# mpkuse/cerebro

Measured on AMD Instinct MI355X. Metric: loop-queries/sec (ticks of 3 descriptors vs 4096-D x 1M DB), higher is better.
Workload: dtype f64

## Files before the change

### cerebro_amd/csrc/chip_api.hip

```cpp
#include "chip_internal.h"
#include <cmath>
#include <cstdlib>
#include <cstring>
#include <memory>
#include <new>

using namespace chip;

extern "C" {

const char *chip_strerror(int status)
{
    switch (status) {
        case CHIP_OK: return "ok";
        case CHIP_ERR_INVALID_ARG: return "invalid argument";
        case CHIP_ERR_NO_DEVICE: return "no usable HIP device";
        case CHIP_ERR_HIP: return "HIP runtime error (see chip_last_hip_error)";
        case CHIP_ERR_OOM: return "out of device memory";
        case CHIP_ERR_NOT_F32: return "descriptor value not exactly representable as float32";
        case CHIP_ERR_NONFINITE: return "NaN/Inf in descriptor";
        case CHIP_ERR_RANGE: return "index / length out of range";
        case CHIP_ERR_UNSUPPORTED: return "unsupported configuration";
        case CHIP_ERR_TOO_FEW_POINTS: return "fewer than 20 correspondences";
        case CHIP_ERR_BUSY: return "async slot busy or empty";
// ... 140 lines not shown
    if (c->s_pnp) (void)hipStreamDestroy(c->s_pnp);
    delete c;
}

void scan_read_knobs(Ctx *c)
{
    c->scan_block = env_int("CHIP_SCAN_BLOCK", 0);
    if (c->scan_block != 256 && c->scan_block != 512 && c->scan_block != 768 && c->scan_block != 1024) c->scan_block = 0;
    c->scan_blocks_per_cu = env_int("CHIP_SCAN_BPC", 2);
    if (c->scan_blocks_per_cu < 1) c->scan_blocks_per_cu = 1;
    c->scan_variant = env_int("CHIP_SCAN_VARIANT", 0);
    c->scan_rows = env_int("CHIP_SCAN_ROWS", 0);
    c->scan_claim = env_int("CHIP_SCAN_CLAIM", -1);
    c->tick_same_stream = env_int("CHIP_TICK_SAME_STREAM", 1) != 0;
    c->scan_short_bpc = env_int("CHIP_SCAN_SHORT_BPC", 1);
    c->scan_plain_bytes = (double)env_int("CHIP_SCAN_PLAIN_MIB", 768) * 1024 * 1024;
    c->scan_half_bytes = (double)env_int("CHIP_SCAN_HALF_MIB", 192) * 1024 * 1024;
    c->scan_sync_plain_bytes = (double)env_int("CHIP_SCAN_SYNC_PLAIN_MIB", 4096) * 1024 * 1024;
    c->scan_overlap_bytes = (double)env_int("CHIP_SCAN_OVERLAP_GIB", 8) * 1024 * 1024 * 1024;
    c->scan_reserve = env_int("CHIP_SCAN_RESERVE", c->nranks > 1 ? 4 : 0);
    c->max_grid = 512;
    c->scan_streams = env_int("CHIP_SCAN_STREAMS", c->nranks > 1 ? 2 : 4);
    c->tick_fused = env_int("CHIP_TICK_FUSED", 1) != 0;
}

static int create_impl(chip_ctx *c, int64_t capacity_hint, int elem)
{
    hipDeviceProp_t prop;
    CHIP_HIP(c, hipGetDeviceProperties(&prop, c->device));
    c->n_cus = prop.multiProcessorCount;
    std::strncpy(c->arch, prop.gcnArchName, sizeof(c->arch) - 1);
    if (std::strncmp(c->arch, "gfx950", 6) != 0 && !std::getenv("CHIP_ALLOW_ANY_ARCH")) return CHIP_ERR_NO_DEVICE;

    c->segs.reserve(kMaxSegs);

    CHIP_HIP(c, hipStreamCreateWithFlags(&c->s_query, hipStreamNonBlocking));
    CHIP_HIP(c, hipStreamCreateWithFlags(&c->s_append, hipStreamNonBlocking));
    CHIP_HIP(c, hipStreamCreateWithFlags(&c->s_pnp, hipStreamNonBlocking));
    int rc = c->seg_table_dev.alloc(c, kMaxSegs);
    if (rc == CHIP_OK) rc = configure_storage(c, elem);
    if (rc != CHIP_OK) return rc;
    c->stage_bytes = 64ull << 20;
    if (c->stage_bytes < (size_t)c->D * 8 * 64) c->stage_bytes = (size_t)c->D * 8 * 64;
    rc = c->stage_dev.alloc(c, c->stage_bytes);
    if (rc == CHIP_OK) rc = c->flags_dev.alloc(c, 1);
    if (rc == CHIP_OK) rc = c->flags_host.alloc(c, 1);
// ... 333 lines not shown
    scan_args_db(c, &a);
    a.K = K;
    a.partial = c->partial_dev[b];
    for (int t = 0; t < T; t++) {
        a.k[t] = parked[t].k;
        if (a.k[t] > a.n_rows) a.n_rows = a.k[t];
        for (int i = 0; i < 3; i++) a.q[3 * t + i] = parked[t].q[i];
    }
    const int grid = scan_multi_grid(c);
    double E = 0.0;
    int e = 0;
    if (prefilter) {
        std::lock_guard<std::mutex> lk(c->mu);
        if (halfq) {
            e = halfq_exponent(c->row_norm_max);
            a.q_up = std::ldexp(1.0f, e);
            a.s_up = std::ldexp(1.0, e);
            a.s_down = std::ldexp(1.0, -e);
            E = halfq_error_bound(c->D, c->row_norm_max, e);
        } else {
            E = prefilter_error_bound(c->D, c->row_norm_max);
        }
    }
    if (hipEventQuery(c->ev_merged[b]) != hipSuccess) CHIP_HIP(c, hipStreamWaitEvent(c->s_scan, c->ev_merged[b], 0));
    hipEvent_t e1 = nullptr;
    int rc = c->prof_on ? prof_begin(c, c->s_scan, (double)a.n_rows * c->D * c->elem, &e1) : CHIP_OK;
    if (rc == CHIP_OK)
        rc = halfq ? launch_scan_halfq(c, c->s_scan, a, grid) : prefilter ? launch_scan_prefilter(c, c->s_scan, a, grid) : launch_scan_multi(c, c->s_scan, a, T, grid);
    if (rc != CHIP_OK) return rc;
    if (e1) CHIP_HIP(c, hipEventRecord(e1, c->s_scan));
    CHIP_HIP(c, hipEventRecord(c->ev_scan[b], c->s_scan));
    c->pass_ev = c->ev_scan[b];
    c->pass_shared = true;
    c->pass_no++;
    CHIP_HIP(c, hipStreamWaitEvent(c->s_query, c->ev_scan[b], 0));
    chip_topk_entry *exact = c->partial_dev[b] + (size_t)kPassMaxTicks * grid * 3 * K;
    if (prefilter) {
        RescoreArgs ra{};
        ra.seg_table = a.seg_table; ra.seg_shift = a.seg_shift; ra.seg_mask = a.seg_mask; ra.D = a.D; ra.K = K;
        ra.in = c->partial_dev[b]; ra.n_lists = grid; ra.wpb = 8;
        ra.E = E;
        ra.out = exact;
        for (int t = 0; t < T; t++) {
            const Ctx::ParkedTick &pt = parked[t];
            Slot &s = *pt.slot;
            ra.k[t] = pt.k;
            for (int i = 0; i < 3; i++) { ra.q[3 * t + i] = s.pf_q[i] = pt.q[i]; s.cert_host[i] = 0; }
            ra.cert[t] = s.cert_dev;
            s.prefilter = true; s.pf_k = pt.k; s.pf_p = pt.p;
        }
        rc = launch_rescore(c, c->s_query, ra, T);
        if (rc != CHIP_OK) return rc;
        Ctx::LastPass &lp = c->last_pass;
        lp.family = halfq ? CHIP_SCAN_FAMILY_HALFQ : CHIP_SCAN_FAMILY_PREFILTER;
        lp.ticks = T; lp.grid = grid; lp.wpb = ra.wpb; lp.K = K; lp.e = e; lp.ring = b; lp.E = E;
        for (int t = 0; t < T; t++) { lp.k[t] = parked[t].k; lp.cert[t] = parked[t].slot->cert_host; }
    }
    if (halfq) {
        PassMergeArgs m{};
        m.in = exact;
        m.K = K;
        for (int t = 0; t < T; t++) {
            const MergeArgs mt = merge_args(exact + (size_t)t * 3 * K, 1, K, nullptr, parked[t].slot->rec.dev(), parked[t].l, &parked[t].p);
            m.result[t] = mt.result; m.l[t] = mt.l; m.locality[t] = mt.locality; m.thresh[t] = mt.thresh;
        }
        rc = launch_pass_merge(c, c->s_query, m, T);
        if (rc != CHIP_OK) return rc;
    }
    for (int t = 0; t < T; t++) {
        const Ctx::ParkedTick &pt = parked[t];
        if (halfq) rc = CHIP_OK;
        else if (prefilter) rc = launch_merge(c, c->s_query, merge_args(exact + (size_t)t * 3 * K, 1, K, nullptr, pt.slot->rec.dev(), pt.l, &pt.p), 3);
        else rc = launch_merge(c, c->s_query, merge_args(c->partial_dev[b] + (size_t)t * grid * 3 * K, grid, K, nullptr, pt.slot->rec.dev(), pt.l, &pt.p), 3);
        if (rc != CHIP_OK) return rc;
        CHIP_HIP(c, hipEventRecord(pt.slot->done, c->s_query));
        pt.slot->wait_ev = pt.slot->done;
        pt.slot->state = SlotState::Event;
        pt.slot->pass_no = c->pass_no;
    }
    CHIP_HIP(c, hipEventRecord(c->ev_merged[b], c->s_query));
    c->coalesce_passes++;
    c->coalesce_ticks += T;
    if (prefilter) { c->prefilter_passes++; c->prefilter_ticks += T; }
    return CHIP_OK;
}

int coalesce_flush(Ctx *c)
{
    const int T = c->n_parked;
    if (T == 0) return CHIP_OK;
    c->n_parked = 0;
    const Ctx::ParkedTick &p0 = c->parked[0];
    int rc;
    if (T == kHalfqTicks && !scan_halfq_usable(c)) {
        rc = coalesce_submit(c, 0, kMultiMaxTicks);
        if (rc == CHIP_OK) rc = coalesce_submit(c, kMultiMaxTicks, T - kMultiMaxTicks);
    } else if (T == kPrefilterTicks && !scan_prefilter_usable(c)) {
        const Ctx::ParkedTick &pl = c->parked[T - 1];
        rc = coalesce_submit(c, 0, T - 1);
        if (rc == CHIP_OK) rc = tick_submit(c, pl.k, pl.l, &pl.p, pl.q, false, *pl.slot);
    } else {
        rc = T == 1 ? tick_submit(c, p0.k, p0.l, &p0.p, p0.q, false, *p0.slot) : coalesce_submit(c, 0, T);
    }
// ... 927 lines not shown
```

### cerebro_amd/csrc/chip_internal.h

```cpp
#pragma once
#include <hip/hip_runtime.h>
#include <cstdint>
#include <mutex>
#include <utility>
#include <condition_variable>
#include <vector>
#include "../../include/cerebro_hip.h"

namespace chip {

constexpr int kWave = 64;
constexpr int kMaxSegs = 4096;
constexpr int64_t kSegBytesTarget = 512ll << 20;

struct ScanArgs {
    const void *const *seg_table;
    int32_t seg_shift;
    int64_t seg_mask;
    int64_t n_rows;
    int32_t D;
    int32_t K;
    const void *q[CHIP_MAX_NQ];
    int64_t idx_mul, idx_add;
    chip_topk_entry *partial;
// ... 21 lines not shown
    uint64_t seq_ptr;
    uint64_t seq_val;
    uint32_t dyn_claim;
    uint32_t tail;
};
static_assert(sizeof(ResidentCmd) == 64, "one cache line, one PCIe read");
constexpr uint32_t kResidentLeave = 0xffffffffu;

struct ResidentArgs {
    ScanArgs base;
    const uint32_t *cmd_host;
    uint32_t *cmd_dev;
    unsigned long long *exit_host;
    unsigned long long instance;
    unsigned long long lease_ticks;
    uint32_t done;
    uint32_t direct;
};

constexpr int kMultiMaxTicks = 3;
constexpr int kPrefilterTicks = 4;
constexpr int kRescoreCap = 32;
constexpr int kHalfqTicks = 5;
constexpr int kPassMaxTicks = kHalfqTicks;
struct PassArgs {
    const void *const *seg_table;
    int32_t seg_shift;
    int64_t seg_mask;
    int64_t n_rows;
    int32_t D;
    int32_t K;
    int64_t k[kPassMaxTicks];
    const void *q[3 * kPassMaxTicks];
    chip_topk_entry *partial;
    float q_up;
    double s_down, s_up;
};
struct RescoreArgs {
    const void *const *seg_table;
    int32_t seg_shift;
    int64_t seg_mask;
    int32_t D;
    int32_t K;
    const chip_topk_entry *in;
    int32_t n_lists;
    int32_t wpb;
    int64_t k[kPassMaxTicks];
    const void *q[3 * kPassMaxTicks];
    double E;
    chip_topk_entry *out;
    uint32_t *cert[kPassMaxTicks];
};
struct PassMergeArgs {
    const chip_topk_entry *in;
    int32_t K;
    chip_tick_result *result[kPassMaxTicks];
    int64_t l[kPassMaxTicks];
    int32_t locality[kPassMaxTicks];
    double thresh[kPassMaxTicks];
// ... 218 lines not shown

    DevBuf<char> stage_dev;
    size_t stage_bytes = 0;
    DevBuf<uint32_t> flags_dev;
    PinnedBuf<uint32_t> flags_host;
    DevBuf<unsigned long long> norm2_dev;
    PinnedBuf<unsigned long long> norm2_host;
    double row_norm_max = 0.0;

    static constexpr int kRing = 64;
    hipStream_t s_scan = nullptr;
    hipStream_t s_scan2 = nullptr;
    hipStream_t s_scan_x[2] = {};
    uint64_t n_same_stream = 0;
    DevBuf<chip_topk_entry> partial_dev[kRing];
    int32_t partial_lists[kRing] = {};
    hipEvent_t ev_scan[kRing] = {};
    hipEvent_t ev_merged[kRing] = {};
    DevBuf<int32_t> tickets_dev;
    PinnedBuf<unsigned long long> seq_all;
    unsigned long long tick_seq = 0;
    bool tick_poll = true;
    bool tick_fused = true;
    Resident res;
    uint64_t n_enqueued = 0;
    int32_t max_grid = 0;
    PinnedBuf<chip_topk_entry> topk;

    DevBuf<char> qvec_dev;
    DevBuf<double> scores_dev;
    DevBuf<unsigned long long> stamps_dev;

    std::vector<char> qconv;
    int64_t cap_hint = 0;
    int32_t group_transport = 0;
    mutable int last_comm = 0;
    int32_t comm_init_abandoned = 0;
    Exchange *xchg = nullptr;
    Group *group = nullptr;
    Ctx *parent = nullptr;
    Slot slots[CHIP_MAX_INFLIGHT];
    int64_t last_l = 0;

    struct ParkedTick { Slot *slot; int64_t k, l; chip_dot_params p; const void *q[3]; };
    int32_t coalesce_max = 5;
    bool coalesce_force = false;
// ... 239 lines not shown
```

### cerebro_amd/csrc/kernels.hip

```cpp
#include "chip_internal.h"
#include "topk_merge.h"
#include <cmath>
#include <type_traits>

namespace chip {

typedef float f32x4 __attribute__((ext_vector_type(4)));
typedef double f64x2 __attribute__((ext_vector_type(2)));

template <typename T> struct Vec16;
template <> struct Vec16<float> { typedef f32x4 type; static constexpr int N = 4; };
template <> struct Vec16<double> { typedef f64x2 type; static constexpr int N = 2; };

template <typename V>
__device__ __forceinline__ const __attribute__((address_space(1))) V *as_global(const V *p)
{
    return (const __attribute__((address_space(1))) V *)p;
}

template <typename V>
__device__ __forceinline__ V stream_load(const V *p)
{
    return __builtin_nontemporal_load(as_global(p));
}
// ... 90 lines not shown
template <typename T>
__device__ __forceinline__ const T *row_base(const ScanArgs &a, int64_t r)
{
    return static_cast<const T *>(a.seg_table[r >> a.seg_shift]) + (r & a.seg_mask) * (int64_t)a.D;
}

__device__ __forceinline__ void wave_topk_offer(double s, int64_t gi, int K, int lane, double &my_s, int64_t &my_i, double &thr_s, int64_t &thr_i)
{
    if (key_gt(s, gi, thr_s, thr_i)) {
        const bool worse = key_gt(s, gi, my_s, my_i);
        const unsigned long long m = __ballot(worse) & ((1ull << K) - 1ull);
        const int pos = __builtin_ctzll(m);
        const double up_s = __shfl_up(my_s, 1, 64);
        const int64_t up_i = __shfl_up(my_i, 1, 64);
        if (lane < K) {
            if (lane > pos) { my_s = up_s; my_i = up_i; }
            else if (lane == pos) { my_s = s; my_i = gi; }
        }
        thr_s = __shfl(my_s, K - 1, 64);
        thr_i = __shfl(my_i, K - 1, 64);
    }
}

template <int NQ, typename OutOf>
__device__ __forceinline__ void block_merge_cand(const chip_topk_entry *cand, int K, int lane, int wave, int wpb, OutOf out_of)
{
    __syncthreads();
    for (int q = wave; q < NQ; q += wpb) {
        const int ncand = wpb * K;
        double cs[4];
        int64_t ci[4];
#pragma unroll
        for (int h = 0; h < 4; h++) {
            const int c = lane + 64 * h;
            if (c < ncand) {
                const chip_topk_entry t = cand[((c / K) * NQ + q) * K + (c % K)];
                cs[h] = t.score;
                ci[h] = t.idx;
            } else { cs[h] = -INFINITY; ci[h] = -1; }
        }
        chip_topk_entry *outp = out_of(q);
        for (int j = 0; j < K; j++) {
            double bs = cs[0];
            int64_t bi = ci[0];
#pragma unroll
            for (int h = 1; h < 4; h++)
                if (key_gt(cs[h], ci[h], bs, bi)) { bs = cs[h]; bi = ci[h]; }
#pragma unroll
            for (int m = 32; m >= 1; m >>= 1) {
                const double os = __shfl_xor(bs, m, 64);
                const int64_t oi = __shfl_xor(bi, m, 64);
                if (key_gt(os, oi, bs, bi)) { bs = os; bi = oi; }
            }
#pragma unroll
            for (int h = 0; h < 4; h++)
                if (ci[h] == bi && cs[h] == bs) { cs[h] = -INFINITY; ci[h] = -1; }
            if (lane == 0) { chip_topk_entry t; t.score = bs; t.idx = bi; outp[j] = t; }
        }
    }
}

template <int NQ, typename OutOf>
__device__ __forceinline__ void block_merge_store(char *smem, const double (&my_s)[NQ], const int64_t (&my_i)[NQ],
                                                  int K, int lane, int wave, int wpb, OutOf out_of)
{
    __syncthreads();
    chip_topk_entry *cand = reinterpret_cast<chip_topk_entry *>(smem);
    if (lane < K) {
#pragma unroll
        for (int q = 0; q < NQ; q++) {
            chip_topk_entry t;
            t.score = my_s[q];
            t.idx = my_i[q];
            cand[(wave * NQ + q) * K + lane] = t;
        }
    }
    block_merge_cand<NQ>(cand, K, lane, wave, wpb, out_of);
}

template <typename T, typename Args>
// ... 44 lines not shown
    __syncthreads();

    double my_s[NQ], thr_s[NQ];
    int64_t my_i[NQ], thr_i[NQ];
#pragma unroll
    for (int q = 0; q < NQ; q++) { my_s[q] = -INFINITY; my_i[q] = -1; thr_s[q] = -INFINITY; thr_i[q] = -1; }

    const int64_t tw = (int64_t)gridDim.x * wpb;
    for (int64_t r = (int64_t)blockIdx.x * wpb + wave; r < a.n_rows; r += tw) {
        const T *row[1] = {row_base<T>(a, r)};
        double acc[1][NQ];
        rows_dot<T, NQ, U, FULL, NT, 1>(row, qs, D, lane, acc);
#pragma unroll
        for (int q = 0; q < NQ; q++) acc[0][q] = butterfly_sum(acc[0][q]);
        const int64_t gi = r * a.idx_mul + a.idx_add;
#pragma unroll
        for (int q = 0; q < NQ; q++) wave_topk_offer(acc[0][q], gi, K, lane, my_s[q], my_i[q], thr_s[q], thr_i[q]);
    }

    block_merge_store<NQ>(smem, my_s, my_i, K, lane, wave, wpb, [&](int q) { return a.partial + ((int64_t)blockIdx.x * NQ + q) * K; });
}

constexpr int kMultiR = 4, kMultiU = 4, kMultiBlock = 512;

constexpr int kMultiVgprBase = 192;
#if defined(__HIP_DEVICE_COMPILE__) && !defined(__gfx950__)
#error "the shared-pass kernels name physical VGPRs: gfx950 (MI355X) only -- build with --offload-arch=gfx950"
#endif
#define CHIP_PASS_SLOTS_192_255                                                                                                         \
    "v192", "v193", "v194", "v195", "v196", "v197", "v198", "v199", "v200", "v201", "v202", "v203", "v204", "v205", "v206", "v207",     \
    "v208", "v209", "v210", "v211", "v212", "v213", "v214", "v215", "v216", "v217", "v218", "v219", "v220", "v221", "v222", "v223",     \
    "v224", "v225", "v226", "v227", "v228", "v229", "v230", "v231", "v232", "v233", "v234", "v235", "v236", "v237", "v238", "v239",     \
    "v240", "v241", "v242", "v243", "v244", "v245", "v246", "v247", "v248", "v249", "v250", "v251", "v252", "v253", "v254", "v255"
#define CHIP_PASS_SLOTS_160_191                                                                                                         \
    "v160", "v161", "v162", "v163", "v164", "v165", "v166", "v167", "v168", "v169", "v170", "v171", "v172", "v173", "v174", "v175",     \
    "v176", "v177", "v178", "v179", "v180", "v181", "v182", "v183", "v184", "v185", "v186", "v187", "v188", "v189", "v190", "v191"
#define CHIP_PASS_SLOTS_144_159                                                                                                         \
    "v144", "v145", "v146", "v147", "v148", "v149", "v150", "v151", "v152", "v153", "v154", "v155", "v156", "v157", "v158", "v159"
__host__ __device__ constexpr int pass_row_slot(int u, int rr) { return kMultiVgprBase + 4 * (u * kMultiR + rr); }
__host__ __device__ constexpr int pass_query_slot(int ng, int u, int g) { return kMultiVgprBase - 4 * kMultiU * ng + 4 * (u * ng + g); }
__host__ __device__ constexpr int pass_vgpr_base(int max_ng) { return kMultiVgprBase - 4 * kMultiU * max_ng; }

template <int N, int I = 0, class F>
__device__ __forceinline__ void static_for(F &&f)
{
    if constexpr (I < N) {
// ... 137 lines not shown
            if (lane > pos) me = up;
            else if (lane == pos) { me.score = s; me.idx = gi; }
            list[lane] = me;
        }
        if constexpr (SCALED) thr_s = (S)(readlane_f64(me.score, K - 1) * sc_up);
        else thr_s = (S)readlane_f64(me.score, K - 1);
    }
}

template <typename T, int NS>
__device__ __forceinline__ void pass_stage_copy(T *qs, const PassArgs &a, int tid)
{
    typedef typename Vec16<T>::type V;
    constexpr int N = Vec16<T>::N;
    const int D = a.D;
    for (int e = tid * N; e < D; e += blockDim.x * N) {
        V w[NS];
#pragma unroll
        for (int q = 0; q < NS; q++) w[q] = *as_global(reinterpret_cast<const V *>(static_cast<const T *>(a.q[q]) + e));
#pragma unroll
        for (int q = 0; q < NS; q++) *reinterpret_cast<V *>(qs + q * D + e) = w[q];
    }
}

template <class P>
__device__ __forceinline__ void shared_pass(const PassArgs &a)
{
    typedef typename P::Elem T;
    typedef typename P::Score S;
    typedef typename P::Staged Q;
    constexpr int NQ = P::NQ, NG = P::NG, NS = NQ - NG, R = kMultiR, U = kMultiU, N = Vec16<T>::N;
    constexpr int BATCH = 64 * N * U;
    static_assert(pass_vgpr_base(NG) >= P::kVgprBase && pass_row_slot(U - 1, R - 1) + 4 <= 256, "load slots inside the asm's share of the register file");
    static_assert(NG >= 0 && NS >= 2 && P::L == U * (R + NG) && P::L <= 64, "at least two staged queries (the LDS read-ahead), vmcnt counts to 63");
    extern __shared__ __attribute__((aligned(16))) char smem[];
    asm volatile("" ::: CHIP_PASS_SLOTS_192_255);
    if constexpr (P::kVgprBase <= 160) asm volatile("" ::: CHIP_PASS_SLOTS_160_191);
    if constexpr (P::kVgprBase <= 144) asm volatile("" ::: CHIP_PASS_SLOTS_144_159);
    Q *qs = reinterpret_cast<Q *>(smem);
    const int D = a.D;
    const int K = a.K;
    const int tid = threadIdx.x;
    const int lane = tid & 63;
    const int wave = __builtin_amdgcn_readfirstlane(tid >> 6);
    const int wpb = blockDim.x >> 6;

// ... 67 lines not shown
            if (hit) {
#pragma unroll
                for (int q = 0; q < NQ; q++) {
                    asm volatile("" : "+v"(s[q]));
                    if (__ballot(s[q] >= thr_s[q])) {
#pragma unroll
                        for (int rr = 0; rr < R; rr++) {
                            const int64_t r = rbase + ((int64_t)group * R + rr) * tw;
                            if (r < a.n_rows && r < a.k[q / 3]) pass_offer<S, P::kScaled>(lane_value(s[q], 16 * rr), r, K, lane, mylists + q * K, thr_s[q], P::kScaled ? a.s_down : 1.0, P::kScaled ? a.s_up : 1.0);
                        }
                    }
                }
            }
#pragma unroll
            for (int rr = 0; rr < R; rr++)
#pragma unroll
                for (int q = 0; q < NQ; q++) acc[rr][q] = P::zero();
            b = 0;
            group++;
        }
    }
    asm volatile("s_waitcnt vmcnt(0)" ::: "memory");

    block_merge_cand<NQ>(lists, K, lane, wave, wpb,
                         [&](int q) { return a.partial + (((int64_t)(q / 3) * gridDim.x + blockIdx.x) * 3 + q % 3) * K; });
}

constexpr int kSharedMaxNG = 2;
constexpr int kSharedF64MaxTicks = 2;
template <typename T, int NTICKS, int NG_, int MAX_NG>
struct PassF64 {
    typedef T Elem;
    typedef T Staged;
    typedef double Score;
    typedef double Acc;
    static constexpr bool kScaled = false;
    static constexpr int NQ = 3 * NTICKS, NG = NG_, NS = NQ - NG, R = kMultiR, U = kMultiU, L = U * (R + NG), kVgprBase = pass_vgpr_base(MAX_NG);
    static __device__ __forceinline__ void stage(T *qs, const PassArgs &a, int tid) { pass_stage_copy<T, NS>(qs, a, tid); }
    static __device__ __forceinline__ Acc zero() { return 0.0; }
    static __device__ __forceinline__ double lane_sum(Acc v) { return v; }
    static __device__ __forceinline__ void batch(Acc (&acc)[R][NQ], const T *qv, int D, uint32_t voff, const T *const (&row)[R], const T *const (&qg)[NG > 0 ? NG : 1])
    {
        typedef typename Vec16<T>::type V;
        constexpr int N = Vec16<T>::N, SS = U * NS;
        V w[SS];
        w[0] = *reinterpret_cast<const V *>(qv);
        w[1] = *reinterpret_cast<const V *>(qv + D);
        double x[R][N];
        static_for<U * NQ>([&](auto sc) CHIP_INLINE_LAMBDA {
            constexpr int u = sc / NQ, q = sc % NQ;
            if constexpr (q == 0)
                static_for<R>([&](auto rr) CHIP_INLINE_LAMBDA {
                    slot_take<pass_row_slot(u, rr), L - 1>(x[rr]);
                    slot_issue<pass_row_slot(u, rr), u * 1024, true>(voff, row[rr]);
                });
            double wd[N];
            if constexpr (q < NS) {
                constexpr int i = u * NS + q;
                if constexpr (i + 2 < SS) w[i + 2] = *reinterpret_cast<const V *>(qv + ((i + 2) % NS) * D + ((i + 2) / NS) * (64 * N));
// ... 25 lines not shown
    shared_pass<PassF64<double, NTICKS, NG, kSharedMaxNG>>(a);
}

constexpr int kPrefilterMaxNG = 3;
typedef float f32x2 __attribute__((ext_vector_type(2)));

template <int REG>
__device__ __forceinline__ void prefilter_fma(f32x2 &acc, f32x2 w)
{
    asm volatile("v_pk_fma_f32 %0, v[%2:%3], %1, %0" : "+v"(acc) : "v"(w), "n"(REG), "n"(REG + 1));
}
template <int REG, int QREG>
__device__ __forceinline__ void prefilter_fma_slot(f32x2 &acc)
{
    asm volatile("v_pk_fma_f32 %0, v[%1:%2], v[%3:%4], %0" : "+v"(acc) : "n"(REG), "n"(REG + 1), "n"(QREG), "n"(QREG + 1));
}

template <int NG_>
struct PassF32 {
    typedef float Elem;
    typedef float Staged;
    typedef float Score;
    typedef f32x2 Acc;
    static constexpr bool kScaled = false;
    static constexpr int NQ = 3 * kPrefilterTicks, NG = NG_, NS = NQ - NG, R = kMultiR, U = kMultiU, L = U * (R + NG), kVgprBase = pass_vgpr_base(kPrefilterMaxNG);
    static __device__ __forceinline__ void stage(float *qs, const PassArgs &a, int tid) { pass_stage_copy<float, NS>(qs, a, tid); }
    static __device__ __forceinline__ Acc zero() { return (f32x2){0.0f, 0.0f}; }
    static __device__ __forceinline__ float lane_sum(Acc v) { return v[0] + v[1]; }
    static __device__ __forceinline__ void batch(Acc (&acc)[R][NQ], const float *qv, int D, uint32_t voff, const float *const (&row)[R], const float *const (&qg)[NG > 0 ? NG : 1])
    {
        constexpr int SS = U * NS;
        f32x4 w[SS];
        w[0] = *reinterpret_cast<const f32x4 *>(qv);
        w[1] = *reinterpret_cast<const f32x4 *>(qv + D);
        static_for<U>([&](auto uc) CHIP_INLINE_LAMBDA {
            constexpr int u = uc;
            slot_wait<L - R>();
            static_for<NS>([&](auto qc) CHIP_INLINE_LAMBDA {
                constexpr int q = qc, i = u * NS + q;
                if constexpr (i + 2 < SS) w[i + 2] = *reinterpret_cast<const f32x4 *>(qv + ((i + 2) % NS) * D + ((i + 2) / NS) * 256);
                const f32x2 wl = __builtin_shufflevector(w[i], w[i], 0, 1), wh = __builtin_shufflevector(w[i], w[i], 2, 3);
                static_for<R>([&](auto rr) CHIP_INLINE_LAMBDA { prefilter_fma<pass_row_slot(u, rr)>(acc[rr][q], wl); });
                static_for<R>([&](auto rr) CHIP_INLINE_LAMBDA { prefilter_fma<pass_row_slot(u, rr) + 2>(acc[rr][q], wh); });
                __builtin_amdgcn_sched_barrier(0);
            });
            static_for<NG>([&](auto gc) CHIP_INLINE_LAMBDA {
                constexpr int g = gc, QR = pass_query_slot(NG, u, g);
                slot_wait<L - R - 1 - g>();
                static_for<R>([&](auto rr) CHIP_INLINE_LAMBDA { prefilter_fma_slot<pass_row_slot(u, rr), QR>(acc[rr][NS + g]); });
                static_for<R>([&](auto rr) CHIP_INLINE_LAMBDA { prefilter_fma_slot<pass_row_slot(u, rr) + 2, QR + 2>(acc[rr][NS + g]); });
            });
            slots_issue_kib<u, NG>(voff, row, qg);
        });
    }
};

template <int NG>
__global__ __launch_bounds__(kMultiBlock) __attribute__((amdgpu_num_vgpr(pass_vgpr_base(kPrefilterMaxNG) / 2))) void db_scan_prefilter(PassArgs a)
{
    static_assert(NG <= kPrefilterMaxNG, "the compiler's share is sized for kPrefilterMaxNG query slots per KiB");
    shared_pass<PassF32<NG>>(a);
}

typedef _Float16 f16x4 __attribute__((ext_vector_type(4)));
struct PassF32H {
    typedef float Elem;
    typedef _Float16 Staged;
    typedef float Score;
    typedef f32x2 Acc;
    static constexpr bool kScaled = true;
    static constexpr int NQ = 3 * kHalfqTicks, NG = 0, NS = NQ, R = kMultiR, U = kMultiU, L = U * R, kVgprBase = pass_vgpr_base(0);
    static __device__ __forceinline__ void stage(_Float16 *qs, const PassArgs &a, int tid)
    {
        const int D = a.D;
        const float up = a.q_up;
        for (int e = tid * 4; e < D; e += blockDim.x * 4) {
            f32x4 w[NS];
#pragma unroll
            for (int q = 0; q < NS; q++) w[q] = *as_global(reinterpret_cast<const f32x4 *>(static_cast<const float *>(a.q[q]) + e));
#pragma unroll
            for (int q = 0; q < NS; q++) {
                f16x4 h;
#pragma unroll
                for (int c = 0; c < 4; c++) h[c] = (_Float16)(w[q][c] * up);
                *reinterpret_cast<f16x4 *>(qs + q * D + e) = h;
            }
        }
    }
    static __device__ __forceinline__ Acc zero() { return (f32x2){0.0f, 0.0f}; }
    static __device__ __forceinline__ float lane_sum(Acc v) { return v[0] + v[1]; }
    static __device__ __forceinline__ void batch(Acc (&acc)[R][NQ], const _Float16 *qv, int D, uint32_t voff, const float *const (&row)[R], const float *const (&qg)[1])
    {
        constexpr int SS = U * NS;
// ... 1 lines not shown
        w[0] = *reinterpret_cast<const f16x4 *>(qv);
        w[1] = *reinterpret_cast<const f16x4 *>(qv + D);
        static_for<U>([&](auto uc) CHIP_INLINE_LAMBDA {
            constexpr int u = uc;
            slot_wait<L - R>();
            static_for<NS>([&](auto qc) CHIP_INLINE_LAMBDA {
                constexpr int q = qc, i = u * NS + q;
                if constexpr (i + 2 < SS) w[i + 2] = *reinterpret_cast<const f16x4 *>(qv + ((i + 2) % NS) * D + ((i + 2) / NS) * 256);
                const f32x2 wl = {(float)w[i][0], (float)w[i][1]}, wh = {(float)w[i][2], (float)w[i][3]};
                static_for<R>([&](auto rr) CHIP_INLINE_LAMBDA { prefilter_fma<pass_row_slot(u, rr)>(acc[rr][q], wl); });
                static_for<R>([&](auto rr) CHIP_INLINE_LAMBDA { prefilter_fma<pass_row_slot(u, rr) + 2>(acc[rr][q], wh); });
                __builtin_amdgcn_sched_barrier(0);
            });
            slots_issue_kib<u, 0>(voff, row, qg);
        });
    }
};

__global__ __launch_bounds__(kMultiBlock) __attribute__((amdgpu_num_vgpr(pass_vgpr_base(0) / 2))) void db_scan_halfq(PassArgs a)
{
    shared_pass<PassF32H>(a);
}

__device__ __forceinline__ void block_best(double &bs, int64_t &bi, double *red_s, int64_t *red_i, int lane, int wave)
{
#pragma unroll
    for (int m = 32; m >= 1; m >>= 1) {
        const double os = __shfl_xor(bs, m, 64);
        const int64_t oi = __shfl_xor(bi, m, 64);
        if (key_gt(os, oi, bs, bi)) { bs = os; bi = oi; }
    }
    __syncthreads();
    if (lane == 0) { red_s[wave] = bs; red_i[wave] = bi; }
    __syncthreads();
    bs = red_s[0]; bi = red_i[0];
#pragma unroll
    for (int w = 1; w < 8; w++)
        if (key_gt(red_s[w], red_i[w], bs, bi)) { bs = red_s[w]; bi = red_i[w]; }
}

__global__ __launch_bounds__(512) void tick_rescore(RescoreArgs a)
{
    constexpr int MAXH = 512 * CHIP_MAX_TOPK / 512;
    __shared__ double red_s[8];
    __shared__ int64_t red_i[8];
    __shared__ chip_topk_entry cand[kRescoreCap];
    __shared__ int n_cand;
    const int tid = threadIdx.x, lane = tid & 63;
    const int wave = __builtin_amdgcn_readfirstlane(tid >> 6);
    const int tick = blockIdx.x / 3, q = blockIdx.x % 3;
    const int K = a.K, n = a.n_lists * K;
    const chip_topk_entry *in = a.in + (int64_t)tick * a.n_lists * 3 * K;
    const int64_t k = a.k[tick];
    if (tid == 0) n_cand = 0;
    double es[MAXH];
    int64_t ei[MAXH];
#pragma unroll
    for (int h = 0; h < MAXH; h++) {
        const int c = tid + 512 * h;
        es[h] = -INFINITY; ei[h] = -1;
        if (c < n) { const chip_topk_entry t = in[((int64_t)(c / K) * 3 + q) * K + (c % K)]; es[h] = t.score; ei[h] = t.idx; }
    }
    double ms = -INFINITY;
    int64_t mi = -1;
    const int64_t tw = (int64_t)a.n_lists * a.wpb;
#pragma unroll
    for (int h = 0; h < MAXH; h++) {
        const int c = tid + 512 * h;
        if (c % K != K - 1 || ei[h] < 0) continue;
        int64_t part = k % tw - (int64_t)(c / K) * a.wpb;
        part = part < 0 ? 0 : part > a.wpb ? a.wpb : part;
        if ((k / tw) * a.wpb + part > K && es[h] > ms) { ms = es[h]; mi = 0; }
    }
    block_best(ms, mi, red_s, red_i, lane, wave);
    double gs = INFINITY;
    int64_t gi = INT64_MAX;
    for (int j = 0; j < K; j++) {
        double bs = -INFINITY;
        int64_t bi = -1;
#pragma unroll
        for (int h = 0; h < MAXH; h++)
            if (key_gt(gs, gi, es[h], ei[h]) && key_gt(es[h], ei[h], bs, bi)) { bs = es[h]; bi = ei[h]; }
        block_best(bs, bi, red_s, red_i, lane, wave);
        gs = bs; gi = bi;
    }
    double thr = gs - 2.0 * a.E;
    thr -= fabs(thr) * 0x1p-51;
    const bool ok = mi < 0 || ms < thr;
#pragma unroll
    for (int h = 0; h < MAXH; h++)
        if (ei[h] >= 0 && es[h] >= thr) {
            const int at = atomicAdd(&n_cand, 1);
            if (at < kRescoreCap) { chip_topk_entry t; t.score = es[h]; t.idx = ei[h]; cand[at] = t; }
        }
    __syncthreads();
    const int nc = n_cand < kRescoreCap ? n_cand : kRescoreCap;
    const float *qrow = static_cast<const float *>(a.q[3 * tick + q]);
    for (int j = wave; j < nc; j += 8) {
        const int64_t r = cand[j].idx;
        const float *row[1] = {static_cast<const float *>(a.seg_table[r >> a.seg_shift]) + (r & a.seg_mask) * (int64_t)a.D};
        double acc[1][1];
        rows_dot<float, 1, 4, true, 1, 1>(row, qrow, a.D, lane, acc);
        const double s = butterfly_sum(acc[0][0]);
        if (lane == 0) cand[j].score = s;
    }
    __syncthreads();
    if (wave == 0) {
        static_assert(kRescoreCap <= 64, "one lane per candidate");
        chip_topk_entry *out = a.out + (int64_t)(3 * tick + q) * K;
        chip_topk_entry me;
        me.score = -INFINITY; me.idx = -1;
        if (lane < nc) me = cand[lane];
        int rank = 0;
        for (int j = 0; j < nc; j++) {
            const chip_topk_entry o = cand[j];
            rank += key_gt(o.score, o.idx, me.score, me.idx) ? 1 : 0;
        }
        if (lane < nc && rank < K) out[rank] = me;
        if (lane >= nc && lane < K) out[lane] = me;
        if (lane == 0) a.cert[tick][q] = ok && n_cand <= kRescoreCap ? 1u : 2u;
    }
}

template <int NQ, int NG, bool FULL>
__global__ __launch_bounds__(1024) void db_scan_topk_wide(ScanArgs a)
{
    static_assert(NG >= 1 && NG < NQ, "at least one query staged, at least one read in place");
    extern __shared__ __attribute__((aligned(16))) char smem[];
    double *qs = reinterpret_cast<double *>(smem);
    constexpr int NL = NQ - NG, U = 4, CH = 128;
    const int D = a.D, K = a.K;
    const int tid = threadIdx.x, lane = tid & 63;
    const int wave = __builtin_amdgcn_readfirstlane(tid >> 6);
    const int wpb = blockDim.x >> 6;
    stage_queries<double, NL>(a, qs, tid, blockDim.x);
    __syncthreads();
    const double *qg[NG];
#pragma unroll
    for (int g = 0; g < NG; g++) qg[g] = static_cast<const double *>(a.q[NL + g]);

    double my_s[NQ], thr_s[NQ];
    int64_t my_i[NQ], thr_i[NQ];
#pragma unroll
// ... 26 lines not shown
                }
            }
        }
#pragma unroll
        for (int q = 0; q < NQ; q++) acc[q] = butterfly_sum(acc[q]);
        const int64_t gi = r * a.idx_mul + a.idx_add;
#pragma unroll
        for (int q = 0; q < NQ; q++) wave_topk_offer(acc[q], gi, K, lane, my_s[q], my_i[q], thr_s[q], thr_i[q]);
    }
    block_merge_store<NQ>(smem, my_s, my_i, K, lane, wave, wpb, [&](int q) { return a.partial + ((int64_t)blockIdx.x * NQ + q) * K; });
}

__device__ __forceinline__ uint32_t lds_byte_addr(const void *p)
{
    return (uint32_t)(uintptr_t)(const __attribute__((address_space(3))) void *)p;
}
__device__ __forceinline__ void glds16_q(const void *gsrc_lane, uint32_t lds_base_wave_uniform)
{
    unsigned keep;
    asm volatile("s_mov_b32 %0, m0\n\ts_mov_b32 m0, %2\n\ts_nop 0\n\tglobal_load_lds_dwordx4 %1, off\n\ts_mov_b32 m0, %0"
                 : "=&s"(keep)
                 : "v"(gsrc_lane), "s"(lds_base_wave_uniform)
                 : "memory");
}

__device__ __forceinline__ void store_entry_agent(chip_topk_entry *p, double s, int64_t i)
{
    __hip_atomic_store(reinterpret_cast<unsigned long long *>(&p->score), (unsigned long long)__double_as_longlong(s), __ATOMIC_RELAXED, __HIP_MEMORY_SCOPE_AGENT);
    __hip_atomic_store(reinterpret_cast<unsigned long long *>(&p->idx), (unsigned long long)i, __ATOMIC_RELAXED, __HIP_MEMORY_SCOPE_AGENT);
}
__device__ __forceinline__ chip_topk_entry load_entry_agent(const chip_topk_entry *p)
{
    chip_topk_entry e;
    e.score = __longlong_as_double((long long)__hip_atomic_load(reinterpret_cast<const unsigned long long *>(&p->score), __ATOMIC_RELAXED, __HIP_MEMORY_SCOPE_AGENT));
    e.idx = (int64_t)__hip_atomic_load(reinterpret_cast<const unsigned long long *>(&p->idx), __ATOMIC_RELAXED, __HIP_MEMORY_SCOPE_AGENT);
    return e;
}

template <int NQ>
__device__ __forceinline__ void block_merge_lists(const ScanArgs &a, const chip_topk_entry *lists, int K, int lane, int wave, int wpb, bool coherent = false)
{
    __syncthreads();
    for (int q = wave; q < NQ; q += wpb) {
        const int ncand = wpb * K;
        double cs[4];
        int64_t ci[4];
#pragma unroll
        for (int h = 0; h < 4; h++) {
            const int c = lane + 64 * h;
            if (c < ncand) {
                const chip_topk_entry t = lists[((c / K) * NQ + q) * CHIP_MAX_TOPK + (c % K)];
                cs[h] = t.score;
                ci[h] = t.idx;
            } else { cs[h] = -INFINITY; ci[h] = -1; }
        }
        chip_topk_entry *outp = a.partial + ((int64_t)blockIdx.x * NQ + q) * K;
        for (int j = 0; j < K; j++) {
            double bs = cs[0];
            int64_t bi = ci[0];
// ... 828 lines not shown
int launch_scan_multi(Ctx *c, hipStream_t s, const PassArgs &a, int n_ticks, int grid)
{
    chip_debug_scan_launch f;
    if (n_ticks > scan_multi_max_ticks(c) || grid > c->max_grid || scan_multi_plan(c->D, c->elem, n_ticks, a.K, grid, &f) != CHIP_OK)
        return CHIP_ERR_UNSUPPORTED;
    if (c->elem == 4) return n_ticks == 2 ? launch_pass(c, s, db_scan_topk_multi<2>, a, f) : launch_pass(c, s, db_scan_topk_multi<3>, a, f);
    static_assert(kSharedF64MaxTicks == 2 && kSharedMaxNG == 2, "the instantiations below");
    if (f.NG == 0) return launch_pass(c, s, db_scan_shared_f64<2, 0>, a, f);
    if (f.NG == 1) return launch_pass(c, s, db_scan_shared_f64<2, 1>, a, f);
    return launch_pass(c, s, db_scan_shared_f64<2, 2>, a, f);
}

int launch_scan_prefilter(Ctx *c, hipStream_t s, const PassArgs &a, int grid)
{
    chip_debug_scan_launch f;
    if (grid > c->max_grid || scan_prefilter_plan(c->D, c->elem, a.K, grid, &f) != CHIP_OK) return CHIP_ERR_UNSUPPORTED;
    return f.NG == 0 ? launch_pass(c, s, db_scan_prefilter<0>, a, f) : launch_pass(c, s, db_scan_prefilter<kPrefilterMaxNG>, a, f);
}

int launch_scan_halfq(Ctx *c, hipStream_t s, const PassArgs &a, int grid)
{
    chip_debug_scan_launch f;
    if (grid > c->max_grid || scan_halfq_plan(c->D, c->elem, a.K, grid, &f) != CHIP_OK || !(a.q_up > 0.0f)) return CHIP_ERR_UNSUPPORTED;
    return launch_pass(c, s, db_scan_halfq, a, f);
}

int launch_rescore(Ctx *c, hipStream_t s, const RescoreArgs &a, int n_ticks)
{
    if (a.n_lists > 512 || a.K > CHIP_MAX_TOPK || n_ticks < 1 || n_ticks > kPassMaxTicks) return CHIP_ERR_UNSUPPORTED;
    hipLaunchKernelGGL(tick_rescore, dim3(3 * n_ticks), dim3(512), 0, s, a);
    CHIP_HIP(c, hipGetLastError());
    return CHIP_OK;
}

int launch_resident(Ctx *c, hipStream_t s, const ResidentArgs &ra, int grid)
{
#ifdef CHIP_NO_ROWS_FORM
    (void)c; (void)s; (void)ra; (void)grid;
    return CHIP_ERR_UNSUPPORTED;
#else
    int block, bpc;
    scan_shape(c, 3, false, &block, &bpc);
    const size_t lds = scan_lds_bytes(c, 3, 1, block, false, true);
    if (lds + 64 > 160 * 1024 || grid > 512) return CHIP_ERR_UNSUPPORTED;
    return c->elem == 8 ? launch_resident_T<double>(c, s, ra, grid, lds, block) : launch_resident_T<float>(c, s, ra, grid, lds, block);
#endif
// ... 330 lines not shown
```

Measured before the change: 1389.

## Fuse halfq pass rescore and merge into scan kernel via last-block ticket

For the half-precision pass, the scan kernel now writes its per-block partial top-k lists with agent-coherent stores, and the last block to finish, found by an atomic ticket, rescores candidates in FP32, writes exact top-k, certificates and per-tick results. This replaces the separate rescore and pass-merge launches and the cross-stream event wait on the query stream, cutting launch latency and stream synchronization per pass. In exchange, the tail is serialized onto a single workgroup, uses a larger LDS scratch area, and depends on ticket reset correctness across passes.

```diff
diff --git a/cerebro_amd/csrc/chip_api.hip b/cerebro_amd/csrc/chip_api.hip
--- a/cerebro_amd/csrc/chip_api.hip
+++ b/cerebro_amd/csrc/chip_api.hip
@@ -186,6 +186,7 @@
     c->max_grid = 512;
     c->scan_streams = env_int("CHIP_SCAN_STREAMS", c->nranks > 1 ? 2 : 4);
     c->tick_fused = env_int("CHIP_TICK_FUSED", 1) != 0;
+    c->pass_fused = env_int("CHIP_PASS_FUSED", 1) != 0;
 }
 
 static int create_impl(chip_ctx *c, int64_t capacity_hint, int elem)
@@ -565,6 +566,26 @@
             E = prefilter_error_bound(c->D, c->row_norm_max);
         }
     }
+    const bool fused = halfq && c->pass_fused;
+    chip_topk_entry *exact = c->partial_dev[b] + (size_t)kPassMaxTicks * grid * 3 * K;
+    if (prefilter) {
+        for (int t = 0; t < T; t++) {
+            const Ctx::ParkedTick &pt = parked[t];
+            Slot &s = *pt.slot;
+            for (int i = 0; i < 3; i++) { s.pf_q[i] = pt.q[i]; s.cert_host[i] = 0; }
+            s.prefilter = true; s.pf_k = pt.k; s.pf_p = pt.p;
+        }
+    }
+    if (fused) {
+        a.ticket = c->tickets_dev + b;
+        a.E = E;
+        a.exact = exact;
+        for (int t = 0; t < T; t++) {
+            const MergeArgs mt = merge_args(exact + (size_t)t * 3 * K, 1, K, nullptr, parked[t].slot->rec.dev(), parked[t].l, &parked[t].p);
+            a.cert[t] = parked[t].slot->cert_dev;
+            a.result[t] = mt.result; a.l[t] = mt.l; a.locality[t] = mt.locality; a.thresh[t] = mt.thresh;
+        }
+    }
     if (hipEventQuery(c->ev_merged[b]) != hipSuccess) CHIP_HIP(c, hipStreamWaitEvent(c->s_scan, c->ev_merged[b], 0));
     hipEvent_t e1 = nullptr;
     int rc = c->prof_on ? prof_begin(c, c->s_scan, (double)a.n_rows * c->D * c->elem, &e1) : CHIP_OK;
@@ -576,30 +597,30 @@
     c->pass_ev = c->ev_scan[b];
     c->pass_shared = true;
     c->pass_no++;
-    CHIP_HIP(c, hipStreamWaitEvent(c->s_query, c->ev_scan[b], 0));
-    chip_topk_entry *exact = c->partial_dev[b] + (size_t)kPassMaxTicks * grid * 3 * K;
+    hipStream_t s_finish = fused ? c->s_scan : c->s_query;
+    if (!fused) CHIP_HIP(c, hipStreamWaitEvent(c->s_query, c->ev_scan[b], 0));
     if (prefilter) {
+        Ctx::LastPass &lp = c->last_pass;
+        lp.family = halfq ? CHIP_SCAN_FAMILY_HALFQ : CHIP_SCAN_FAMILY_PREFILTER;
+        lp.ticks = T; lp.grid = grid; lp.wpb = kPassWpb; lp.K = K; lp.e = e; lp.ring = b; lp.E = E;
+        for (int t = 0; t < T; t++) { lp.k[t] = parked[t].k; lp.cert[t] = parked[t].slot->cert_host; }
+    }
+    if (prefilter && !fused) {
         RescoreArgs ra{};
         ra.seg_table = a.seg_table; ra.seg_shift = a.seg_shift; ra.seg_mask = a.seg_mask; ra.D = a.D; ra.K = K;
-        ra.in = c->partial_dev[b]; ra.n_lists = grid; ra.wpb = 8;
+        ra.in = c->partial_dev[b]; ra.n_lists = grid; ra.wpb = kPassWpb;
         ra.E = E;
         ra.out = exact;
         for (int t = 0; t < T; t++) {
             const Ctx::ParkedTick &pt = parked[t];
-            Slot &s = *pt.slot;
             ra.k[t] = pt.k;
-            for (int i = 0; i < 3; i++) { ra.q[3 * t + i] = s.pf_q[i] = pt.q[i]; s.cert_host[i] = 0; }
-            ra.cert[t] = s.cert_dev;
-            s.prefilter = true; s.pf_k = pt.k; s.pf_p = pt.p;
+            for (int i = 0; i < 3; i++) ra.q[3 * t + i] = pt.q[i];
+            ra.cert[t] = pt.slot->cert_dev;
         }
         rc = launch_rescore(c, c->s_query, ra, T);
         if (rc != CHIP_OK) return rc;
-        Ctx::LastPass &lp = c->last_pass;
-        lp.family = halfq ? CHIP_SCAN_FAMILY_HALFQ : CHIP_SCAN_FAMILY_PREFILTER;
-        lp.ticks = T; lp.grid = grid; lp.wpb = ra.wpb; lp.K = K; lp.e = e; lp.ring = b; lp.E = E;
-        for (int t = 0; t < T; t++) { lp.k[t] = parked[t].k; lp.cert[t] = parked[t].slot->cert_host; }
-    }
-    if (halfq) {
+    }
+    if (halfq && !fused) {
         PassMergeArgs m{};
         m.in = exact;
         m.K = K;
@@ -616,12 +637,12 @@
         else if (prefilter) rc = launch_merge(c, c->s_query, merge_args(exact + (size_t)t * 3 * K, 1, K, nullptr, pt.slot->rec.dev(), pt.l, &pt.p), 3);
         else rc = launch_merge(c, c->s_query, merge_args(c->partial_dev[b] + (size_t)t * grid * 3 * K, grid, K, nullptr, pt.slot->rec.dev(), pt.l, &pt.p), 3);
         if (rc != CHIP_OK) return rc;
-        CHIP_HIP(c, hipEventRecord(pt.slot->done, c->s_query));
+        CHIP_HIP(c, hipEventRecord(pt.slot->done, s_finish));
         pt.slot->wait_ev = pt.slot->done;
         pt.slot->state = SlotState::Event;
         pt.slot->pass_no = c->pass_no;
     }
-    CHIP_HIP(c, hipEventRecord(c->ev_merged[b], c->s_query));
+    CHIP_HIP(c, hipEventRecord(c->ev_merged[b], s_finish));
     c->coalesce_passes++;
     c->coalesce_ticks += T;
     if (prefilter) { c->prefilter_passes++; c->prefilter_ticks += T; }
diff --git a/cerebro_amd/csrc/chip_internal.h b/cerebro_amd/csrc/chip_internal.h
--- a/cerebro_amd/csrc/chip_internal.h
+++ b/cerebro_amd/csrc/chip_internal.h
@@ -67,6 +67,7 @@
 constexpr int kPrefilterTicks = 4;
 constexpr int kRescoreCap = 32;
 constexpr int kHalfqTicks = 5;
+constexpr int kPassWpb = 8;
 constexpr int kPassMaxTicks = kHalfqTicks;
 struct PassArgs {
     const void *const *seg_table;
@@ -80,6 +81,14 @@
     chip_topk_entry *partial;
     float q_up;
     double s_down, s_up;
+    int32_t *ticket;
+    double E;
+    chip_topk_entry *exact;
+    uint32_t *cert[kPassMaxTicks];
+    chip_tick_result *result[kPassMaxTicks];
+    int64_t l[kPassMaxTicks];
+    int32_t locality[kPassMaxTicks];
+    double thresh[kPassMaxTicks];
 };
 struct RescoreArgs {
     const void *const *seg_table;
@@ -344,6 +353,7 @@
     unsigned long long tick_seq = 0;
     bool tick_poll = true;
     bool tick_fused = true;
+    bool pass_fused = true;
     Resident res;
     uint64_t n_enqueued = 0;
     int32_t max_grid = 0;
diff --git a/cerebro_amd/csrc/kernels.hip b/cerebro_amd/csrc/kernels.hip
--- a/cerebro_amd/csrc/kernels.hip
+++ b/cerebro_amd/csrc/kernels.hip
@@ -136,8 +136,21 @@
     }
 }
 
+__device__ __forceinline__ void store_entry_agent(chip_topk_entry *p, double s, int64_t i)
+{
+    __hip_atomic_store(reinterpret_cast<unsigned long long *>(&p->score), (unsigned long long)__double_as_longlong(s), __ATOMIC_RELAXED, __HIP_MEMORY_SCOPE_AGENT);
+    __hip_atomic_store(reinterpret_cast<unsigned long long *>(&p->idx), (unsigned long long)i, __ATOMIC_RELAXED, __HIP_MEMORY_SCOPE_AGENT);
+}
+__device__ __forceinline__ chip_topk_entry load_entry_agent(const chip_topk_entry *p)
+{
+    chip_topk_entry e;
+    e.score = __longlong_as_double((long long)__hip_atomic_load(reinterpret_cast<const unsigned long long *>(&p->score), __ATOMIC_RELAXED, __HIP_MEMORY_SCOPE_AGENT));
+    e.idx = (int64_t)__hip_atomic_load(reinterpret_cast<const unsigned long long *>(&p->idx), __ATOMIC_RELAXED, __HIP_MEMORY_SCOPE_AGENT);
+    return e;
+}
+
 template <int NQ, typename OutOf>
-__device__ __forceinline__ void block_merge_cand(const chip_topk_entry *cand, int K, int lane, int wave, int wpb, OutOf out_of)
+__device__ __forceinline__ void block_merge_cand(const chip_topk_entry *cand, int K, int lane, int wave, int wpb, OutOf out_of, bool coherent = false)
 {
     __syncthreads();
     for (int q = wave; q < NQ; q += wpb) {
@@ -169,7 +182,10 @@
 #pragma unroll
             for (int h = 0; h < 4; h++)
                 if (ci[h] == bi && cs[h] == bs) { cs[h] = -INFINITY; ci[h] = -1; }
-            if (lane == 0) { chip_topk_entry t; t.score = bs; t.idx = bi; outp[j] = t; }
+            if (lane == 0) {
+                if (coherent) store_entry_agent(outp + j, bs, bi);
+                else { chip_topk_entry t; t.score = bs; t.idx = bi; outp[j] = t; }
+            }
         }
     }
 }
@@ -260,6 +276,7 @@
 }
 
 constexpr int kMultiR = 4, kMultiU = 4, kMultiBlock = 512;
+static_assert(kMultiBlock == 64 * kPassWpb, "tick_rescore and pass_finish count a workgroup's rows with kPassWpb");
 
 constexpr int kMultiVgprBase = 192;
 #if defined(__HIP_DEVICE_COMPILE__) && !defined(__gfx950__)
@@ -443,6 +460,9 @@
         for (int q = 0; q < NS; q++) *reinterpret_cast<V *>(qs + q * D + e) = w[q];
     }
 }
+
+template <int NT>
+__device__ __forceinline__ void pass_finish(const PassArgs &a, char *smem, int K, int tid, int lane, int wave, int wpb);
 
 template <class P>
 __device__ __forceinline__ void shared_pass(const PassArgs &a)
@@ -556,8 +576,12 @@
     }
     asm volatile("s_waitcnt vmcnt(0)" ::: "memory");
 
+    bool finish = false;
+    if constexpr (P::kFinish) finish = a.ticket != nullptr;
     block_merge_cand<NQ>(lists, K, lane, wave, wpb,
-                         [&](int q) { return a.partial + (((int64_t)(q / 3) * gridDim.x + blockIdx.x) * 3 + q % 3) * K; });
+                         [&](int q) { return a.partial + (((int64_t)(q / 3) * gridDim.x + blockIdx.x) * 3 + q % 3) * K; }, finish);
+    if constexpr (P::kFinish)
+        if (finish) pass_finish<NQ / 3>(a, smem, K, tid, lane, wave, wpb);
 }
 
 constexpr int kSharedMaxNG = 2;
@@ -568,7 +592,7 @@
     typedef T Staged;
     typedef double Score;
     typedef double Acc;
-    static constexpr bool kScaled = false;
+    static constexpr bool kScaled = false, kFinish = false;
     static constexpr int NQ = 3 * NTICKS, NG = NG_, NS = NQ - NG, R = kMultiR, U = kMultiU, L = U * (R + NG), kVgprBase = pass_vgpr_base(MAX_NG);
     static __device__ __forceinline__ void stage(T *qs, const PassArgs &a, int tid) { pass_stage_copy<T, NS>(qs, a, tid); }
     static __device__ __forceinline__ Acc zero() { return 0.0; }
@@ -640,7 +664,7 @@
     typedef float Staged;
     typedef float Score;
     typedef f32x2 Acc;
-    static constexpr bool kScaled = false;
+    static constexpr bool kScaled = false, kFinish = false;
     static constexpr int NQ = 3 * kPrefilterTicks, NG = NG_, NS = NQ - NG, R = kMultiR, U = kMultiU, L = U * (R + NG), kVgprBase = pass_vgpr_base(kPrefilterMaxNG);
     static __device__ __forceinline__ void stage(float *qs, const PassArgs &a, int tid) { pass_stage_copy<float, NS>(qs, a, tid); }
     static __device__ __forceinline__ Acc zero() { return (f32x2){0.0f, 0.0f}; }
@@ -686,7 +710,7 @@
     typedef _Float16 Staged;
     typedef float Score;
     typedef f32x2 Acc;
-    static constexpr bool kScaled = true;
+    static constexpr bool kScaled = true, kFinish = true;
     static constexpr int NQ = 3 * kHalfqTicks, NG = 0, NS = NQ, R = kMultiR, U = kMultiU, L = U * R, kVgprBase = pass_vgpr_base(0);
     static __device__ __forceinline__ void stage(_Float16 *qs, const PassArgs &a, int tid)
     {
@@ -734,6 +758,52 @@
     shared_pass<PassF32H>(a);
 }
 
+__device__ __forceinline__ int64_t pass_rows_owned(int64_t k, int64_t tw, int b, int wpb)
+{
+    int64_t part = k % tw - (int64_t)b * wpb;
+    part = part < 0 ? 0 : part > wpb ? wpb : part;
+    return (k / tw) * wpb + part;
+}
+__device__ __forceinline__ double rescore_threshold(double G, double E)
+{
+    double thr = G - 2.0 * E;
+    thr -= fabs(thr) * 0x1p-51;
+    return thr;
+}
+template <int NR, class Args>
+__device__ __forceinline__ void rescore_rows(const Args &a, const float *qrow, chip_topk_entry *cand, int j0, int nc, int lane)
+{
+    const float *row[NR];
+#pragma unroll
+    for (int rr = 0; rr < NR; rr++) {
+        const int64_t r = cand[j0 + rr < nc ? j0 + rr : j0].idx;
+        row[rr] = static_cast<const float *>(a.seg_table[r >> a.seg_shift]) + (r & a.seg_mask) * (int64_t)a.D;
+    }
+    double acc[NR][1];
+    rows_dot<float, 1, 4, true, 1, NR>(row, qrow, a.D, lane, acc);
+#pragma unroll
+    for (int rr = 0; rr < NR; rr++) {
+        const double s = butterfly_sum(acc[rr][0]);
+        if (lane == 0 && j0 + rr < nc) cand[j0 + rr].score = s;
+    }
+}
+template <class Put>
+__device__ __forceinline__ void rescore_write(const chip_topk_entry *cand, int nc, int K, int lane, bool certified, uint32_t *cert, Put put)
+{
+    static_assert(kRescoreCap <= 64, "one lane per candidate");
+    chip_topk_entry me;
+    me.score = -INFINITY; me.idx = -1;
+    if (lane < nc) me = cand[lane];
+    int rank = 0;
+    for (int j = 0; j < nc; j++) {
+        const chip_topk_entry o = cand[j];
+        rank += key_gt(o.score, o.idx, me.score, me.idx) ? 1 : 0;
+    }
+    if (lane < nc && rank < K) put(rank, me);
+    if (lane >= nc && lane < K) put(lane, me);
+    if (lane == 0) *cert = certified ? 1u : 2u;
+}
+
 __device__ __forceinline__ void block_best(double &bs, int64_t &bi, double *red_s, int64_t *red_i, int lane, int wave)
 {
 #pragma unroll
@@ -780,9 +850,7 @@
     for (int h = 0; h < MAXH; h++) {
         const int c = tid + 512 * h;
         if (c % K != K - 1 || ei[h] < 0) continue;
-        int64_t part = k % tw - (int64_t)(c / K) * a.wpb;
-        part = part < 0 ? 0 : part > a.wpb ? a.wpb : part;
-        if ((k / tw) * a.wpb + part > K && es[h] > ms) { ms = es[h]; mi = 0; }
+        if (pass_rows_owned(k, tw, c / K, a.wpb) > K && es[h] > ms) { ms = es[h]; mi = 0; }
     }
     block_best(ms, mi, red_s, red_i, lane, wave);
     double gs = INFINITY;
@@ -796,8 +864,7 @@
         block_best(bs, bi, red_s, red_i, lane, wave);
         gs = bs; gi = bi;
     }
-    double thr = gs - 2.0 * a.E;
-    thr -= fabs(thr) * 0x1p-51;
+    const double thr = rescore_threshold(gs, a.E);
     const bool ok = mi < 0 || ms < thr;
 #pragma unroll
     for (int h = 0; h < MAXH; h++)
@@ -808,29 +875,140 @@
     __syncthreads();
     const int nc = n_cand < kRescoreCap ? n_cand : kRescoreCap;
     const float *qrow = static_cast<const float *>(a.q[3 * tick + q]);
-    for (int j = wave; j < nc; j += 8) {
-        const int64_t r = cand[j].idx;
-        const float *row[1] = {static_cast<const float *>(a.seg_table[r >> a.seg_shift]) + (r & a.seg_mask) * (int64_t)a.D};
-        double acc[1][1];
-        rows_dot<float, 1, 4, true, 1, 1>(row, qrow, a.D, lane, acc);
-        const double s = butterfly_sum(acc[0][0]);
-        if (lane == 0) cand[j].score = s;
-    }
+    for (int j = wave; j < nc; j += 8) rescore_rows<1>(a, qrow, cand, j, nc, lane);
     __syncthreads();
     if (wave == 0) {
-        static_assert(kRescoreCap <= 64, "one lane per candidate");
         chip_topk_entry *out = a.out + (int64_t)(3 * tick + q) * K;
-        chip_topk_entry me;
-        me.score = -INFINITY; me.idx = -1;
-        if (lane < nc) me = cand[lane];
-        int rank = 0;
-        for (int j = 0; j < nc; j++) {
-            const chip_topk_entry o = cand[j];
-            rank += key_gt(o.score, o.idx, me.score, me.idx) ? 1 : 0;
-        }
-        if (lane < nc && rank < K) out[rank] = me;
-        if (lane >= nc && lane < K) out[lane] = me;
-        if (lane == 0) a.cert[tick][q] = ok && n_cand <= kRescoreCap ? 1u : 2u;
+        rescore_write(cand, nc, K, lane, ok && n_cand <= kRescoreCap, &a.cert[tick][q], [&](int rank, const chip_topk_entry &e) { out[rank] = e; });
+    }
+}
+
+__device__ __forceinline__ chip_tick_result single_list_record(const chip_topk_entry (&top)[3], int64_t l, int locality, double thresh)
+{
+    chip_tick_result res;
+    res.status = CHIP_TICK_SCANNED;
+    res.found = 0;
+    res.idx_curr = -1;
+    res.idx_prev = -1;
+    res.score = 0.0;
+    for (int q = 0; q < 3; q++) {
+        res.argmax[q] = top[q].idx >= 0 ? top[q].idx : -1;
+        res.maxv[q] = top[q].idx >= 0 ? top[q].score : -INFINITY;
+    }
+    if (res.argmax[0] >= 0 && res.argmax[1] >= 0 && res.argmax[2] >= 0) {
+        int64_t d1 = res.argmax[0] - res.argmax[1];
+        int64_t d2 = res.argmax[0] - res.argmax[2];
+        if (d1 < 0) d1 = -d1;
+        if (d2 < 0) d2 = -d2;
+        if (d1 < locality && d2 < locality && res.maxv[0] > thresh) {
+            res.found = 1;
+            res.idx_curr = l - 1;
+            res.idx_prev = res.argmax[0];
+            res.score = res.maxv[0];
+        }
+    }
+    return res;
+}
+
+constexpr int kFinishCandOff = 256, kFinishSortedOff = kFinishCandOff + 3 * kPassMaxTicks * kRescoreCap * (int)sizeof(chip_topk_entry);
+constexpr int kFinishSmem = kFinishSortedOff + 3 * kPassMaxTicks * CHIP_MAX_TOPK * (int)sizeof(chip_topk_entry);
+template <int NT>
+__device__ __forceinline__ void pass_finish(const PassArgs &a, char *smem, int K, int tid, int lane, int wave, int wpb)
+{
+    constexpr int NP = 3 * NT, CH = 16, NR = 4;
+    static_assert(NP <= 3 * kPassMaxTicks && 4 * NP <= 64 && kRescoreCap % NR == 0, "the scratch map above");
+    int *last = reinterpret_cast<int *>(smem);
+    int *n_cand = reinterpret_cast<int *>(smem + 64);
+    int *cert_ok = reinterpret_cast<int *>(smem + 128);
+    chip_topk_entry *cand = reinterpret_cast<chip_topk_entry *>(smem + kFinishCandOff);
+    chip_topk_entry *sorted = reinterpret_cast<chip_topk_entry *>(smem + kFinishSortedOff);
+    asm volatile("s_waitcnt vmcnt(0)" ::: "memory");
+    __syncthreads();
+    if (tid == 0) *last = __hip_atomic_fetch_add(a.ticket, 1, __ATOMIC_RELAXED, __HIP_MEMORY_SCOPE_AGENT) == (int)gridDim.x - 1;
+    __syncthreads();
+    if (!*last) return;
+    __builtin_amdgcn_fence(__ATOMIC_ACQUIRE, "agent");
+    if (tid == 0) __hip_atomic_store(a.ticket, 0, __ATOMIC_RELAXED, __HIP_MEMORY_SCOPE_AGENT);
+
+    const int n_lists = (int)gridDim.x, n = n_lists * K;
+    const int64_t tw = (int64_t)n_lists * wpb;
+#pragma unroll 1
+    for (int p = wave; p < NP; p += wpb) {
+        const chip_topk_entry *in = a.partial + ((int64_t)(p / 3) * n_lists * 3 + p % 3) * K;
+        const int64_t k = a.k[p / 3];
+        auto load = [&](chip_topk_entry (&e)[CH], int c0) {
+#pragma unroll
+            for (int h = 0; h < CH; h++) {
+                const int c = c0 + 64 * h + lane;
+                e[h].score = -INFINITY; e[h].idx = -1;
+                if (c < n) e[h] = load_entry_agent(in + (int64_t)(c / K) * 3 * K + c % K);
+            }
+        };
+        double my_s = -INFINITY, gs = -INFINITY;
+        int64_t my_i = -1, gi = -1;
+        chip_topk_entry e[CH];
+#pragma unroll 1
+        for (int c0 = 0; c0 < n; c0 += 64 * CH) {
+            load(e, c0);
+#pragma unroll
+            for (int h = 0; h < CH; h++) {
+                unsigned long long m = __ballot(e[h].idx >= 0 && key_gt(e[h].score, e[h].idx, gs, gi));
+                while (m) {
+                    const int l = __builtin_ctzll(m);
+                    m &= m - 1;
+                    wave_topk_offer(readlane_f64(e[h].score, l), readlane_i64(e[h].idx, l), K, lane, my_s, my_i, gs, gi);
+                }
+            }
+        }
+        const double thr = rescore_threshold(gs, a.E);
+        double ms = -INFINITY;
+        bool dropped = false;
+        int cnt = 0;
+        chip_topk_entry *mine = cand + p * kRescoreCap;
+#pragma unroll 1
+        for (int c0 = 0; c0 < n; c0 += 64 * CH) {
+            if (n > 64 * CH) load(e, c0);
+#pragma unroll
+            for (int h = 0; h < CH; h++) {
+                const int c = c0 + 64 * h + lane;
+                const bool valid = e[h].idx >= 0;
+                if (valid && c % K == K - 1 && pass_rows_owned(k, tw, c / K, wpb) > K && e[h].score > ms) { ms = e[h].score; dropped = true; }
+                const bool in_r = valid && e[h].score >= thr;
+                const unsigned long long m = __ballot(in_r);
+                const int at = cnt + __popcll(m & ((1ull << lane) - 1ull));
+                if (in_r && at < kRescoreCap) mine[at] = e[h];
+                cnt += __popcll(m);
+            }
+        }
+#pragma unroll
+        for (int m = 32; m >= 1; m >>= 1) {
+            const double o = __shfl_xor(ms, m, 64);
+            ms = o > ms ? o : ms;
+        }
+        const bool ok = __ballot(dropped) == 0ull || ms < thr;
+        if (lane == 0) { n_cand[p] = cnt; cert_ok[p] = ok ? 1 : 0; }
+    }
+    __syncthreads();
+#pragma unroll 1
+    for (int g = wave; g < NP * (kRescoreCap / NR); g += wpb) {
+        const int p = g % NP, j0 = (g / NP) * NR;
+        const int nc = n_cand[p] < kRescoreCap ? n_cand[p] : kRescoreCap;
+        if (j0 < nc) rescore_rows<NR>(a, static_cast<const float *>(a.q[p]), cand + p * kRescoreCap, j0, nc, lane);
+    }
+    __syncthreads();
+#pragma unroll 1
+    for (int p = wave; p < NP; p += wpb) {
+        const int nc = n_cand[p] < kRescoreCap ? n_cand[p] : kRescoreCap;
+        chip_topk_entry *out = a.exact + (int64_t)p * K, *lout = sorted + p * K;
+        rescore_write(cand + p * kRescoreCap, nc, K, lane, cert_ok[p] != 0 && n_cand[p] <= kRescoreCap, a.cert[p / 3] + p % 3,
+                      [&](int rank, const chip_topk_entry &e) { out[rank] = e; lout[rank] = e; });
+    }
+    __syncthreads();
+    if (tid < NT) {
+        chip_topk_entry top[3];
+#pragma unroll
+        for (int q = 0; q < 3; q++) top[q] = sorted[(3 * tid + q) * K];
+        *a.result[tid] = single_list_record(top, a.l[tid], a.locality[tid], a.thresh[tid]);
     }
 }
 
@@ -903,19 +1081,6 @@
                  : "=&s"(keep)
                  : "v"(gsrc_lane), "s"(lds_base_wave_uniform)
                  : "memory");
-}
-
-__device__ __forceinline__ void store_entry_agent(chip_topk_entry *p, double s, int64_t i)
-{
-    __hip_atomic_store(reinterpret_cast<unsigned long long *>(&p->score), (unsigned long long)__double_as_longlong(s), __ATOMIC_RELAXED, __HIP_MEMORY_SCOPE_AGENT);
-    __hip_atomic_store(reinterpret_cast<unsigned long long *>(&p->idx), (unsigned long long)i, __ATOMIC_RELAXED, __HIP_MEMORY_SCOPE_AGENT);
-}
-__device__ __forceinline__ chip_topk_entry load_entry_agent(const chip_topk_entry *p)
-{
-    chip_topk_entry e;
-    e.score = __longlong_as_double((long long)__hip_atomic_load(reinterpret_cast<const unsigned long long *>(&p->score), __ATOMIC_RELAXED, __HIP_MEMORY_SCOPE_AGENT));
-    e.idx = (int64_t)__hip_atomic_load(reinterpret_cast<const unsigned long long *>(&p->idx), __ATOMIC_RELAXED, __HIP_MEMORY_SCOPE_AGENT);
-    return e;
 }
 
 template <int NQ>
@@ -1790,6 +1955,7 @@
 {
     chip_debug_scan_launch f;
     if (grid > c->max_grid || scan_halfq_plan(c->D, c->elem, a.K, grid, &f) != CHIP_OK || !(a.q_up > 0.0f)) return CHIP_ERR_UNSUPPORTED;
+    if (a.ticket && (f.lds_bytes < kFinishSmem || grid > 512 || a.K > CHIP_MAX_TOPK)) return CHIP_ERR_UNSUPPORTED;
     return launch_pass(c, s, db_scan_halfq, a, f);
 }
 
```

After: 1346. 0.969x the previous value.
